# jialeli1/From-Voxel-to-Point

Hardware: AMD Instinct MI355X
Metric: point clouds/sec fwd+bwd (FV2P, KITTI shape) at 1/2/4/8 MI355X (higher is better)
Workload: dtype f32

## Files before the change

### from-voxel-to-point_amd/csrc_torch/fv2p_torch.cpp

```cpp
#include <torch/extension.h>
#include <c10/hip/HIPStream.h>
#include <c10/hip/HIPGuard.h>
#include <c10/hip/HIPCachingAllocator.h>
#include <c10/core/DeviceGuard.h>
#include <hip/hip_runtime_api.h>

#include <atomic>
#include <cstdlib>

#include <map>
#include <tuple>
#include <vector>
#include <mutex>
#include <string>

#include "../../include/fv2p_ops.h"

namespace {

using torch::autograd::AutogradContext;
using torch::autograd::variable_list;

void* cur_stream(const at::Tensor& t) { return static_cast<void*>(c10::hip::getCurrentHIPStream(t.device().index()).stream()); }

// ... 443 lines not shown
    }
    ctx->save_for_backward({x, mean, invstd, weight.has_value() ? *weight : at::Tensor(), bias.has_value() ? *bias : at::Tensor()});
    ctx->saved_data["relu"] = relu;
    ctx->saved_data["batch_stats"] = batch_stats;
    return y;
  }

  static variable_list backward(AutogradContext* ctx, variable_list grads) {
    const auto saved = ctx->get_saved_variables();
    const at::Tensor &x = saved[0], &mean = saved[1], &invstd = saved[2], &weight = saved[3], &bias = saved[4];
    const at::Tensor dz = grads[0].contiguous();
    const int64_t n = x.size(0), c = x.size(1), hw = x.size(2) * x.size(3);
    c10::DeviceGuard guard(x.device());
    void* stream = cur_stream(x);
    at::Tensor dx = at::empty_like(x);
    at::Tensor dpar = at::empty({2, c}, x.options());
    at::Tensor ws = workspace(fv2p_batchnorm2d_ws_bytes(n, static_cast<int>(c), hw), x, stream);
    check(fv2p_batchnorm2d_backward(x.data_ptr<float>(), dz.data_ptr<float>(), n, static_cast<int>(c), hw, mean.data_ptr<float>(), invstd.data_ptr<float>(),
                                    weight.defined() ? weight.data_ptr<float>() : nullptr, bias.defined() ? bias.data_ptr<float>() : nullptr,
                                    ctx->saved_data["relu"].toBool() ? 1 : 0, ctx->saved_data["batch_stats"].toBool() ? 1 : 0, dx.data_ptr<float>(),
                                    dpar[0].data_ptr<float>(), dpar[1].data_ptr<float>(), ws.data_ptr(), static_cast<size_t>(ws.numel()), stream),
          "fv2p_batchnorm2d_backward");
    return {dx, weight.defined() ? dpar[0] : at::Tensor(), bias.defined() ? dpar[1] : at::Tensor(), at::Tensor(), at::Tensor(), at::Tensor(),
            at::Tensor(), at::Tensor(), at::Tensor(), at::Tensor()};
  }
};

at::Tensor batch_norm2d_relu(const at::Tensor& x, const c10::optional<at::Tensor>& weight, const c10::optional<at::Tensor>& bias,
                             const c10::optional<at::Tensor>& running_mean, const c10::optional<at::Tensor>& running_var,
                             const c10::optional<at::Tensor>& num_batches_tracked, bool training, double momentum, double eps, bool relu) {
  return BnRelu2dFn::apply(x, weight, bias, running_mean, running_var, num_batches_tracked, training, momentum, eps, relu);
}

at::Tensor sparse_conv_bn_relu(const at::Tensor& features, const at::Tensor& weight, const at::Tensor& tab_f, int64_t flip_f, const at::Tensor& tab_b,
                               int64_t flip_b, int64_t n_out, int64_t centre, const c10::optional<at::Tensor>& pairs,
                               const c10::optional<at::Tensor>& pair_num, int64_t side_src, const c10::optional<at::Tensor>& conv_bias,
                               const c10::optional<at::Tensor>& bn_weight, const c10::optional<at::Tensor>& bn_bias,
                               const c10::optional<at::Tensor>& running_mean, const c10::optional<at::Tensor>& running_var,
                               const c10::optional<at::Tensor>& num_batches_tracked, bool training, double momentum, double eps, bool relu,
                               const c10::optional<at::Tensor>& perm_b) {
  if (n_out < 2 && training) return at::Tensor();
  const bool has_bias = conv_bias.has_value() && conv_bias->defined();
  const bool batch_stats = training || !(running_mean.has_value() && running_mean->defined());
  const int64_t cout = weight.size(-1);
  if (fuse_bn_stats() && batch_stats && !has_bias && cout <= 1024 && features.is_cuda()) {
    c10::DeviceGuard guard(features.device());
    StatRing& ring = stat_ring(features, cur_stream(features));
    const int cur = ring.cur, other = 1 - cur;
    at::Tensor y = SparseConvFn::apply(features, weight, tab_f, flip_f, tab_b, flip_b, n_out, centre, pairs, pair_num, side_src,
                                       c10::optional<at::Tensor>(ring.buf[cur]), perm_b);
    ring.dirty[cur] = static_cast<int64_t>(fv2p_sparse_conv_stat_slots()) * 2 * cout;
    at::Tensor out = BnReluFn::apply(y, bn_weight, bn_bias, running_mean, running_var, num_batches_tracked, training, momentum, eps, relu,
                                     c10::optional<at::Tensor>(ring.buf[cur]), c10::optional<at::Tensor>(ring.buf[other]), ring.dirty[other]);
    ring.dirty[other] = 0;
    ring.cur = other;
    return out;
  }
  at::Tensor y = SparseConvFn::apply(features, weight, tab_f, flip_f, tab_b, flip_b, n_out, centre, pairs, pair_num, side_src, c10::optional<at::Tensor>(),
                                     perm_b);
  if (has_bias) y = y + *conv_bias;
  return BnReluFn::apply(y, bn_weight, bn_bias, running_mean, running_var, num_batches_tracked, training, momentum, eps, relu,
                         c10::optional<at::Tensor>(), c10::optional<at::Tensor>(), 0);
}


struct FinState {
// ... 494 lines not shown
  m.def("abi_version", []() { return fv2p_abi_version(); });
  m.def("set_bn_epilogue", &set_bn_epilogue, "BatchNorm sums from the conv epilogues (default) or from BatchNorm's own reduce pass");
  m.def("gate_weights", &gate_weights, "aliases of the conv weights whose gradients are joined from the side stream at the end of backward");
  m.def("sparse_conv", &sparse_conv, "fused sparse convolution with autograd (tables from a Rulebook)");
  m.def("batch_norm_relu", &batch_norm_relu, "BatchNorm1d (+ReLU) on [N, C] with autograd");
  m.def("batch_norm2d_relu", &batch_norm2d_relu, "BatchNorm2d (+ReLU) on a contiguous [N, C, H, W] map with autograd");
  m.def("voxelize_batch_mean", &voxelize_batch_mean, py::arg("clouds"), py::arg("voxel_size"), py::arg("range_lo"), py::arg("grid"),
        py::arg("max_points"), py::arg("max_voxels"), py::arg("cloud_streams") = true, py::call_guard<py::gil_scoped_release>(),
        "voxelise a batch of clouds + MeanVFE + collate, without the GIL");
  m.def("build_rulebook_chain", &build_rulebook_chain, py::call_guard<py::gil_scoped_release>(),
        "build a chain of rulebooks (and pair lists) from root coordinates, without the GIL");
  m.def("conv_fin", &conv_fin, "sparse conv with its BatchNorm statistics finalised by the launch (and optionally the source rows' BatchNorm + ReLU on the gather) -> [y, saved]");
  m.def("bn_apply", &bn_apply, "relu?((x - mean) * invstd * gamma + beta [+ residual]) with finalised statistics, one launch");
  m.def("prenorm_supported", &prenorm_supported, "the conv kernel of this shape can normalise its source rows on the gather");
  m.def("set_bn_fold", &set_bn_fold, "round-6 arrangement of conv / BatchNorm / residual blocks on (default) or off (the round-5 one)");
  m.def("bn_fold", &bn_fold);
  m.def("set_deterministic", &set_deterministic, "deterministic mode: no float-atomic conv-epilogue statistics (BatchNorm's own fixed-order reduce)");
  m.def("deterministic", &deterministic);
  m.def("set_bn_one", &set_bn_one, "BatchNorm passes without conv-epilogue sums as one launch each (default) or as reduce + apply");
  m.def("bn_one", &bn_one);
  m.def("set_bn_wide", &set_bn_wide, "large BatchNorm passes with the wide reduce finalised by its own launch (default) or the <= 64-workgroup reduce + folding apply");
  m.def("bn_wide", &bn_wide);
  m.def("record_entry_points", [](bool on) {
    std::lock_guard<std::mutex> lock(g_record_mu);
    g_entries.clear();
    g_record.store(on);
  }, "log the name of every library entry point the binding calls (tests), and clear the log");
  m.def("entry_points", []() {
    std::lock_guard<std::mutex> lock(g_record_mu);
    std::vector<std::string> out;
    out.swap(g_entries);
    return out;
  }, "the entry points called since the last collection");
  m.def("sparse_conv_bn_relu", &sparse_conv_bn_relu, "sparse conv -> BatchNorm1d (-> ReLU) with autograd, one call per backbone block");
}
```

### from-voxel-to-point_amd/fv2p_harness/fv2p_model.py

```python
import math
import os
from functools import partial

import numpy as np
import torch
import torch.nn as nn
import torch.nn.functional as F

from pcdet.ops.iou3d_nms import iou3d_nms_cuda, iou3d_nms_utils
from pcdet.ops.pointnet2.pointnet2_batch import pointnet2_modules as pn2_batch_modules
from pcdet.ops.pointnet2.pointnet2_batch import fused as pn2_fused
from pcdet.ops.pointnet2.pointnet2_batch import pointnet2_utils as pn2_batch
from pcdet.ops.pointnet2.pointnet2_stack import pointnet2_utils as pn2_stack
from pcdet.ops.roiaware_pool3d import roiaware_pool3d_utils
from pcdet.ops.roipoint_pool3d import roipoint_pool3d_utils
from pcdet.models.backbones_3d.pfe import bev_grid_pooling
from pcdet.ops.spconv import norm as _norm

import fv2p_native as _nat

from .backbone import VoxelResBackBone8x, bn_act

TWO_PI = 2.0 * math.pi


class FV2PConfig:
    point_cloud_range = (0.0, -40.0, -3.0, 70.4, 40.0, 1.0)
    voxel_size = (0.05, 0.05, 0.1)
    grid_size = (1408, 1600, 40)
    max_points_per_voxel, max_voxels = 5, 16000
    num_point_features = 4
    bev_layers, bev_strides, bev_filters = (5, 5), (1, 2), (128, 256)
    bev_up_strides, bev_up_filters = (1, 2), (256, 256)
    anchor_rotations = (0.0, 1.57)
    anchor_classes = (((3.9, 1.6, 1.56), -1.78, 0.6, 0.45), ((0.8, 0.6, 1.73), -0.6, 0.5, 0.35), ((1.76, 0.6, 1.73), -0.6, 0.5, 0.35))
    dir_offset, dir_limit_offset, num_dir_bins = 0.78539, 0.0, 2
    rpn_w = dict(cls=1.0, loc=2.0, dir=0.2)
    num_keypoints = 16384
    decode_levels = (("x_conv4", 8, 128, 256), ("x_conv3", 4, 64, 192), ("x_conv2", 2, 32, 160), ("x_conv1", 1, 16, 128))
    init_source, init_stride, init_channels = "x_conv4", 8, 128
    decoder_out = 128
    point_cls_fc, gt_extra_width, point_cls_weight = (64, 64), (0.2, 0.2, 0.2), 4.0
    nms_pre, nms_post, nms_thresh = 9000, 512, 0.8
    roi_per_image, fg_ratio = 128, 0.5
# ... 437 lines not shown

    def __init__(self, cfg, cin):
        super().__init__()
        self.cfg = cfg
        self.cls_layers = mlp1d(cin, cfg.point_cls_fc, out=1)

    @torch.no_grad()
    def assign(self, key, gt):
        boxes = gt[..., :7].contiguous()
        ext = boxes.clone()
        ext[..., 3:6] += dconst(boxes, tuple(float(v) for v in self.cfg.gt_extra_width), boxes.dtype)
        ext = torch.where((boxes[..., 3:6].abs().sum(-1, keepdim=True) > 0), ext, boxes)
        inside = roiaware_pool3d_utils.points_in_boxes_gpu(key, boxes) >= 0
        near = roiaware_pool3d_utils.points_in_boxes_gpu(key, ext) >= 0
        labels = inside.long()
        labels.masked_fill_(inside ^ near, -1)
        return labels.view(-1)

    def forward(self, key, feats, gt):
        logits = run_rows(self.cls_layers, feats)
        labels = self.assign(key, gt)
        pos = labels > 0
        w = ((labels == 0) | pos).float() / pos.sum().float().clamp_min(1.0)
        loss = sigmoid_focal(logits, pos.float().unsqueeze(-1), w).sum() * self.cfg.point_cls_weight
        return loss, torch.sigmoid(logits).max(dim=-1).values


def rows_linear(x, weight, bias=None):
    w = weight.reshape(weight.shape[0], -1).t().unsqueeze(0).expand(x.shape[0], -1, -1)
    y = torch.bmm(x, w)
    return y if bias is None else y + bias


def sa_msg_grid(sa, xyz, features, centres, rows=None):
    outs = []
    xyz_t = xyz.transpose(1, 2)
    ctr_t = centres.transpose(1, 2)
    for grouper, mlp in zip(sa.groupers, sa.mlps):
        layers = list(mlp)
        w1 = layers[0].weight[:, :, 0, 0]
        idx = pn2_batch.ball_query(grouper.radius, grouper.nsample, xyz, centres)
        tail = layers[1:]
        fusable = (len(tail) == 3 and isinstance(tail[0], nn.ReLU) and isinstance(tail[1], nn.Conv2d) and isinstance(tail[2], nn.ReLU)
                   and tail[1].bias is None and tail[1].weight.shape[:2] == (w1.shape[0], w1.shape[0]) and xyz.is_cuda)
        if fusable:
            if rows is None:
                rows = features.transpose(1, 2).contiguous()
            per_point = rows_linear(rows, w1[:, 3:]) + rows_linear(xyz, w1[:, :3])
            per_centre = rows_linear(centres, w1[:, :3])
            if pn2_fused.supported(per_point, idx):
                outs.append(pn2_fused.sa_grid_max(per_point, per_centre, idx, tail[1].weight[:, :, 0, 0]).transpose(1, 2))
                continue
        if features is None:
            features = rows.transpose(1, 2).contiguous()
        per_point = (torch.matmul(w1[:, 3:], features) + torch.matmul(w1[:, :3], xyz_t)).contiguous()
        per_centre = torch.matmul(w1[:, :3], ctr_t)
        h = pn2_batch.grouping_operation(per_point, idx) - per_centre.unsqueeze(-1)
        for layer in tail:
            h = layer(h)
        outs.append(h.amax(dim=-1))
    return torch.cat(outs, dim=1)


class IoUGuidedRoIHead(nn.Module):

    def __init__(self, cfg):
        super().__init__()
        self.cfg = cfg
        self.bev_grid_pool_layer = bev_grid_pooling.BEVGridPooling(
            type("Cfg", (), dict(IN_CHANNELS=cfg.bev_pool_in, OUT_CHANNELS=cfg.bev_pool_out))(), cfg.point_cloud_range, cfg.voxel_size)
        self.roipoint_pool3d_layer = roipoint_pool3d_utils.RoIPointPool3d(cfg.num_sampled_points, list(cfg.pool_extra_width))
        chans = [5] + list(cfg.xyz_up)
        up = []
        for a, c in zip(chans[:-1], chans[1:]):
            up += [nn.Conv2d(a, c, 1), nn.ReLU()]
        self.xyz_up_layer = nn.Sequential(*up)
        c_out = cfg.xyz_up[-1]
        self.merge_down_layer = nn.Sequential(nn.Conv2d(2 * c_out, c_out, 1), nn.ReLU())
        self.SA_modules = nn.ModuleList([pn2_batch_modules.PointnetSAModuleMSG(
            npoint=cfg.grid_size_roi ** 3, radii=list(cfg.sa_radii), nsamples=list(cfg.sa_nsamples),
            mlps=[[c_out] + list(m) for m in cfg.sa_mlps], use_xyz=True, bn=False)])
        sa_out = sum(m[-1] for m in cfg.sa_mlps)
        g3 = cfg.grid_size_roi ** 3
        layers, pre = [], g3 * (sa_out + cfg.bev_pool_out)
        for k, f in enumerate(cfg.interact_filters):
            layers += [nn.Conv1d(pre, f, 1, bias=False), nn.BatchNorm1d(f), nn.ReLU()]
            if k != len(cfg.interact_filters) - 1 and cfg.dp_ratio > 0:
                layers.append(nn.Dropout(cfg.dp_ratio))
# ... 144 lines not shown

    def prepare(self, bev, prop_scores, prop_boxes, gt, uniforms):
        b = bev.shape[0]
        rois, _ = self.proposals(prop_scores, prop_boxes)
        s_rois, s_gt, s_iou = self.sample_targets(rois, gt, uniforms)
        gt_ct = self.canonical_targets(s_rois, s_gt)
        return dict(rois=rois, s_rois=s_rois, s_gt=s_gt, s_iou=s_iou, gt_ct=gt_ct, **self.roi_streams(bev, s_rois))

    def roi_streams(self, bev, s_rois, bev_stride=8):
        b = bev.shape[0]
        world, local = self.grid_points(s_rois)
        batch_dict = {"batch_size": b, "spatial_features_before_head": bev, "spatial_features_stride": bev_stride}
        g = self.cfg.grid_size_roi
        if KERNEL_GLUE and world.shape[1] == g ** 3:
            column = world.view(world.shape[0], g * g, g, 3)[:, :, 0]
            g_bev = self.bev_grid_pool_layer(batch_dict, column.reshape(b, -1, 3))
            g_bev = g_bev.view(world.shape[0], g * g, 1, -1).expand(-1, -1, g, -1).reshape(world.shape[0], g ** 3, -1)
        else:
            g_bev = self.bev_grid_pool_layer(batch_dict, world.view(b, -1, 3)).view(world.shape[0], world.shape[1], -1)
        g_bev = g_bev.permute(0, 2, 1).contiguous()
        t = dconst(s_rois, _CORNER_SIGNS, s_rois.dtype) / 2
        corners = s_rois.reshape(-1, 7)[:, None, 3:6] * t[None]
        cge = self.cge_inter(self.cge_up(corners.transpose(1, 2).unsqueeze(3).contiguous()).squeeze(-1))
        return dict(local=local, g_bev=g_bev, cge=cge)

    def finish(self, key, feats, scores, prep):
        rois = prep["s_rois"]
        cls, reg = self.predict(key, feats, scores, rois, prep)
        loss = self.losses(rois, prep["s_gt"], prep["gt_ct"], prep["s_iou"], cls, reg[:, 1:], reg[:, :1])
        return loss, {"rois": prep["rois"], "sampled_rois": rois, "roi_iou": prep["s_iou"]}

    def predict(self, key, feats, scores, rois, prep):
        pooled = self.pool_points(key, feats, scores, rois)
        h = pooled[..., 0:5]
        for layer in self.xyz_up_layer:
            h = rows_linear(h, layer.weight, layer.bias) if isinstance(layer, nn.Conv2d) else layer(h)
        h = torch.cat((h, pooled[..., 5:]), dim=2)
        for layer in self.merge_down_layer:
            h = rows_linear(h, layer.weight, layer.bias) if isinstance(layer, nn.Conv2d) else layer(h)
        g_pt = sa_msg_grid(self.SA_modules[0], pooled[..., 0:3].contiguous(), None, prep["local"].contiguous(), rows=h)
        grid = torch.cat((g_pt, prep["g_bev"]), dim=1)
        pc = self.grid_interact_fc_layer(grid.view(grid.shape[0], -1, 1))
        shared = self.feature_fusion(torch.cat((pc, prep["cge"]), dim=1))
        cls = self.cls_layers(shared).squeeze(-1)
        reg = self.reg_layers(shared).squeeze(-1)
        return cls, reg

    @staticmethod
    def reg_losses(rois, gt_src, gt_ct, fg, reg):
        n_fg = fg.sum().clamp_min(1.0)
        r7 = rois.reshape(-1, 7)
        anchor = torch.cat((torch.zeros_like(r7[:, :3]), r7[:, 3:6], torch.zeros_like(r7[:, 6:7])), dim=1)
        target = residual_encode(gt_ct.reshape(-1, gt_ct.shape[-1])[:, :7], anchor)
        loss_reg = (smooth_l1(reg - target, 1.0 / 9.0) * fg[:, None]).sum() / n_fg
        local = residual_decode(reg, anchor)
        world = rotate_z(local.unsqueeze(1), r7[:, 6]).squeeze(1)
        world = torch.cat((world[:, :3] + r7[:, :3], world[:, 3:6], world[:, 6:7] + r7[:, 6:7]), dim=1)
        g = gt_src.reshape(-1, gt_src.shape[-1])[:, :7]
        loss_corner = (corner_loss_lidar(world, g) * fg).sum() / n_fg
        return loss_reg, loss_corner

    def losses(self, rois, gt_src, gt_ct, iou, cls, reg, iou_pred):
        cfg = self.cfg
        iou = iou.view(-1)
        soft = ((iou - cfg.cls_bg) / (cfg.cls_fg - cfg.cls_bg)).clamp(0, 1)
        soft = torch.where(iou > cfg.cls_fg, torch.ones_like(soft), torch.where(iou < cfg.cls_bg, torch.zeros_like(soft), soft))
        loss_cls = F.binary_cross_entropy(torch.sigmoid(cls.view(-1)), soft, reduction="none").mean()
        fg = (iou > cfg.reg_fg).float()
        loss_reg, loss_corner = self.reg_losses(rois, gt_src, gt_ct, fg, reg)
        lab = (iou - 0.5) * 2
        valid = (lab >= (cfg.reg_fg - 0.5) * 2).float()
        loss_iou = (F.smooth_l1_loss(iou_pred.view(-1), lab, reduction="none") * valid).sum() / valid.sum().clamp_min(1.0)
        return loss_cls + loss_reg + loss_corner + loss_iou
# ... 95 lines not shown
```

### include/fv2p_ops.h

```cpp
#ifndef FV2P_OPS_H_
#define FV2P_OPS_H_

#include <stddef.h>
#include <stdint.h>

#ifdef __cplusplus
extern "C" {
#endif

#define FV2P_ABI_VERSION 1

#define FV2P_EINVAL      (-1)
#define FV2P_EWORKSPACE  (-2)
#define FV2P_EHIP        (-3)
#define FV2P_ELIMIT      (-4)

typedef void* fv2p_stream_t;

const char* fv2p_last_error(void);
int fv2p_abi_version(void);

size_t fv2p_scan_ws_bytes(int64_t n);
int fv2p_exclusive_scan_i32(const int* in, int* out, int64_t n, int* total, void* ws, size_t ws_bytes,
                            fv2p_stream_t stream);
// ... 267 lines not shown
                                   void* ws, size_t ws_bytes, fv2p_stream_t stream);
size_t fv2p_group_points_stack_grad_ws_bytes(int m, int c, int nsample);
int fv2p_group_points_stack_grad_gather(int b, int m, int c, int n, int nsample, const float* grad_out, const int* idx,
                                        const int* idx_batch_cnt, const int* features_batch_cnt, float* grad_features, void* ws,
                                        size_t ws_bytes, fv2p_stream_t stream);
size_t fv2p_three_interpolate_batch_grad_ws_bytes(int b, int c, int n, int m);
int fv2p_three_interpolate_batch_grad_gather(int b, int c, int n, int m, const float* grad_out, const int* idx, const float* weight,
                                             float* grad_points, void* ws, size_t ws_bytes, fv2p_stream_t stream);

int fv2p_group_points_stack_h(int b, int m, int c, int n, int nsample, const void* features, const int* features_batch_cnt,
                              const int* idx, const int* idx_batch_cnt, void* out, int dtype, fv2p_stream_t stream);
size_t fv2p_group_points_stack_grad_h_ws_bytes(int m, int c, int nsample);
int fv2p_group_points_stack_grad_h(int b, int m, int c, int n, int nsample, const void* grad_out, const int* idx,
                                   const int* idx_batch_cnt, const int* features_batch_cnt, void* grad_features, int dtype,
                                   void* ws, size_t ws_bytes, fv2p_stream_t stream);
int fv2p_three_interpolate_stack_h(int n, int c, int m, const void* features, const int* idx, const float* weight, void* out,
                                   int dtype, fv2p_stream_t stream);
size_t fv2p_three_interpolate_stack_grad_h_ws_bytes(int n, int c, int m);
int fv2p_three_interpolate_stack_grad_h(int n, int c, int m, const void* grad_out, const int* idx, const float* weight,
                                        void* grad_features, int dtype, void* ws, size_t ws_bytes, fv2p_stream_t stream);

int fv2p_sa_grid_supported(int n, int m, int s, int c);
int fv2p_sa_grid_fwd(const float* per_point, const float* per_centre, const int* idx, const float* w2, int rois, int n, int m,
                     int s, int c, float* out, unsigned char* arg, fv2p_stream_t stream);
size_t fv2p_sa_grid_bwd_ws_bytes(int rois);
int fv2p_sa_grid_bwd(const float* per_point, const float* per_centre, const int* idx, const float* w2, const unsigned char* arg,
                     const float* grad_out, int rois, int n, int m, int s, int c, float* grad_point, float* grad_centre,
                     float* grad_w2, void* ws, size_t ws_bytes, fv2p_stream_t stream);
size_t fv2p_sa_grid_bwd_gather_ws_bytes(int rois, int m, int s);
int fv2p_sa_grid_bwd_gather(const float* per_point, const float* per_centre, const int* idx, const float* w2, const unsigned char* arg,
                            const float* grad_out, int rois, int n, int m, int s, int c, float* grad_point, float* grad_centre,
                            float* grad_w2, void* ws, size_t ws_bytes, fv2p_stream_t stream);

int fv2p_dcn_forward(const float* x_nhwc, const float* wt_oc, const float* bias, const float* offset,
                     const float* mask, int batch, int height, int width, int c_in, int c_out, int h_out,
                     int w_out, int kh, int kw, int sh, int sw, int ph, int pw, int dh, int dw,
                     int deformable_group, float* y_nhwc, fv2p_stream_t stream);
int fv2p_dcn_set_forward_order(int order);
int fv2p_dcn_set_colg_cap(int64_t bytes);
size_t fv2p_dcn_backward_ws_bytes(int batch, int height, int width, int h_out, int w_out, int c_in, int c_out, int kh,
                                  int kw, int deformable_group);
int fv2p_dcn_backward(const float* x_nhwc, const float* wt, const float* offset, const float* mask,
                      const float* dy_nhwc, int batch, int height, int width, int c_in, int c_out, int h_out,
                      int w_out, int kh, int kw, int sh, int sw, int ph, int pw, int dh, int dw,
                      int deformable_group, float* dx_nhwc, float* doffset, float* dmask, float* dwt, void* ws,
                      size_t ws_bytes, fv2p_stream_t stream);
int fv2p_dcn_forward_grouped(const float* x_nhwc, const float* wt_oc, const float* bias, const float* offset,
                             const float* mask, int batch, int height, int width, int c_in, int c_out, int h_out,
                             int w_out, int kh, int kw, int sh, int sw, int ph, int pw, int dh, int dw,
                             int deformable_group, int group, float* y_nhwc, fv2p_stream_t stream);
size_t fv2p_dcn_backward_grouped_ws_bytes(int batch, int height, int width, int h_out, int w_out, int c_in, int c_out, int kh,
                                          int kw, int deformable_group, int group);
int fv2p_dcn_backward_grouped(const float* x_nhwc, const float* wt, const float* offset, const float* mask,
                              const float* dy_nhwc, int batch, int height, int width, int c_in, int c_out, int h_out,
                              int w_out, int kh, int kw, int sh, int sw, int ph, int pw, int dh, int dw,
                              int deformable_group, int group, float* dx_nhwc, float* doffset, float* dmask, float* dwt,
                              void* ws, size_t ws_bytes, fv2p_stream_t stream);

int fv2p_transpose_batched(const float* in, int batch, int64_t rows, int64_t cols, float* out, fv2p_stream_t stream);

int fv2p_deform_psroi_pool_forward(const float* data, const float* rois, const float* trans, int batch, int channels,
                                   int height, int width, int num_rois, int no_trans, float spatial_scale,
                                   int output_dim, int group_size, int pooled_size, int part_size,
                                   int sample_per_part, float trans_std, int num_classes, float* out,
                                   float* top_count, fv2p_stream_t stream);
int fv2p_deform_psroi_pool_backward(const float* grad_out, const float* data, const float* rois, const float* trans,
// ... 90 lines not shown
```

Measured before the change: 105.1.

## Fuse RoI point MLP stack and SA first layers into one MFMA kernel

Adds a HIP kernel pair that runs the RoI-head point MLP chain (xyz_up two layers, merge_down, and both SA-branch first 1x1 convs) per 64-row tile in LDS using fp32 MFMA, with a fused backward that computes all weight and bias gradients via per-block partials and a reduction kernel. The model's predict path uses it when the layer shapes match and feeds the per-point outputs straight into the SA grid op. This removes several bmm launches and the intermediate activation tensors' round trips to memory. In exchange it adds weight-fragment packing per call, a fixed-shape specialization, and a change in gradient summation order.

```diff
diff --git a/from-voxel-to-point_amd/csrc/roi_mlp.hip b/from-voxel-to-point_amd/csrc/roi_mlp.hip
--- /dev/null
+++ b/from-voxel-to-point_amd/csrc/roi_mlp.hip
@@ -0,0 +1,476 @@
+#include "common.hpp"
+
+namespace fv2p {
+namespace {
+
+typedef float f32x4 __attribute__((ext_vector_type(4)));
+
+constexpr int kRmC = 128;
+constexpr int kRmIn = 5 + kRmC;
+constexpr int kRmS = 64;
+constexpr int kRmSLd = 3 + kRmC;
+constexpr int kRmT = 64;
+constexpr int kRmThreads = 512;
+constexpr int kRmParts = 240;
+constexpr int kRmLdF = 132;
+constexpr int kRmLdB = 144;
+
+constexpr int kFragW2 = 0;
+constexpr int kFragW3a = 16384;
+constexpr int kFragW3b = 32768;
+constexpr int kFragS0 = 49152;
+constexpr int kFragS1 = 57344;
+constexpr int kFragFwd = 65536;
+constexpr int kFragS0T = 65536;
+constexpr int kFragS1T = 73728;
+constexpr int kFragW3aT = 81920;
+constexpr int kFragW2T = 98304;
+constexpr int kFragBwd = 114688;
+
+constexpr int kGradW1 = 0;
+constexpr int kGradB1 = 640;
+constexpr int kGradW2 = 768;
+constexpr int kGradB2 = 17152;
+constexpr int kGradW3 = 17280;
+constexpr int kGradB3 = 50048;
+constexpr int kGradS0 = 50176;
+constexpr int kGradS1 = 58560;
+constexpr int kGradFloats = 66944;
+
+struct PackJob {
+  const float* src;
+  int ld, col0, transpose, nb, nj, dst;
+};
+struct PackJobs {
+  PackJob job[9];
+};
+
+__global__ __launch_bounds__(256) void roi_mlp_pack_k(PackJobs jobs, float* __restrict__ image) {
+  const PackJob d = jobs.job[blockIdx.y];
+  const int e = blockIdx.x * 256 + threadIdx.x;
+  if (e >= d.nb * d.nj * 64) return;
+  const int lane = e & 63, bj = e >> 6, b = bj / d.nj, j = bj - b * d.nj;
+  const int i = 16 * b + (lane & 15), k = 16 * j + 4 * (lane >> 4);
+  float v[4];
+#pragma unroll
+  for (int c = 0; c < 4; ++c) v[c] = d.transpose ? d.src[(k + c) * d.ld + d.col0 + i] : d.src[i * d.ld + d.col0 + k + c];
+  *reinterpret_cast<float4*>(image + d.dst + static_cast<size_t>(e) * 4) = make_float4(v[0], v[1], v[2], v[3]);
+}
+
+template <int NBW, int NJ, int UJ, typename X>
+__device__ __forceinline__ void mma_rows(const float* __restrict__ frag, int b0, int lane, X x, f32x4 (&acc)[NBW]) {
+#pragma unroll UJ
+  for (int j = 0; j < NJ; ++j) {
+    const float4 xv = x(j);
+    float4 a[NBW];
+#pragma unroll
+    for (int i = 0; i < NBW; ++i)
+      a[i] = *reinterpret_cast<const float4*>(frag + ((b0 + i) * NJ + j) * 256 + static_cast<unsigned>(lane * 4));
+#pragma unroll
+    for (int i = 0; i < NBW; ++i) acc[i] = __builtin_amdgcn_mfma_f32_16x16x4f32(a[i].x, xv.x, acc[i], 0, 0, 0);
+#pragma unroll
+    for (int i = 0; i < NBW; ++i) acc[i] = __builtin_amdgcn_mfma_f32_16x16x4f32(a[i].y, xv.y, acc[i], 0, 0, 0);
+#pragma unroll
+    for (int i = 0; i < NBW; ++i) acc[i] = __builtin_amdgcn_mfma_f32_16x16x4f32(a[i].z, xv.z, acc[i], 0, 0, 0);
+#pragma unroll
+    for (int i = 0; i < NBW; ++i) acc[i] = __builtin_amdgcn_mfma_f32_16x16x4f32(a[i].w, xv.w, acc[i], 0, 0, 0);
+  }
+}
+
+template <int N>
+__device__ __forceinline__ void zero_acc(f32x4 (&acc)[N]) {
+#pragma unroll
+  for (int i = 0; i < N; ++i) acc[i] = f32x4{0.f, 0.f, 0.f, 0.f};
+}
+
+template <int NBW>
+__device__ __forceinline__ void layer1_row(const float (&x)[5], const float* __restrict__ w1, const float* __restrict__ b1, int b0, int g,
+                                           float* __restrict__ dst) {
+#pragma unroll
+  for (int i = 0; i < NBW; ++i) {
+    const int c0 = 16 * (b0 + i) + 4 * g;
+    float v[4];
+#pragma unroll
+    for (int e = 0; e < 4; ++e) {
+      const float* w = w1 + static_cast<unsigned>((c0 + e) * 5);
+      float z = x[0] * w[0];
+      z = fmaf(x[1], w[1], z);
+      z = fmaf(x[2], w[2], z);
+      z = fmaf(x[3], w[3], z);
+      z = fmaf(x[4], w[4], z);
+      v[e] = fmaxf(z + b1[static_cast<unsigned>(c0 + e)], 0.f);
+    }
+    *reinterpret_cast<float4*>(dst + c0) = make_float4(v[0], v[1], v[2], v[3]);
+  }
+}
+
+template <int NBW>
+__device__ __forceinline__ void store_relu(const f32x4 (&acc)[NBW], const float* __restrict__ bias, int b0, int g, float* __restrict__ dst) {
+#pragma unroll
+  for (int i = 0; i < NBW; ++i) {
+    const int c0 = 16 * (b0 + i) + 4 * g;
+    const float4 b = *reinterpret_cast<const float4*>(bias + static_cast<unsigned>(c0));
+    *reinterpret_cast<float4*>(dst + c0) =
+        make_float4(fmaxf(acc[i][0] + b.x, 0.f), fmaxf(acc[i][1] + b.y, 0.f), fmaxf(acc[i][2] + b.z, 0.f), fmaxf(acc[i][3] + b.w, 0.f));
+  }
+}
+
+__global__ __launch_bounds__(kRmThreads, 4) void roi_point_mlp_fwd_k(long long rows, const float* __restrict__ pooled,
+                                                                      const float* __restrict__ w1, const float* __restrict__ b1,
+                                                                      const float* __restrict__ b2, const float* __restrict__ b3,
+                                                                      const float* __restrict__ s0, const float* __restrict__ s1,
+                                                                      const float* __restrict__ frag, float* __restrict__ out0,
+                                                                      float* __restrict__ out1) {
+  __shared__ __attribute__((aligned(16))) float bufa[kRmT * kRmLdF];
+  __shared__ __attribute__((aligned(16))) float bufb[kRmT * kRmLdF];
+  const int lane = threadIdx.x & 63, wave = threadIdx.x >> 6, row = lane & 15, g = lane >> 4;
+  const int rt = wave & 3, hb = wave >> 2, lr = 16 * rt + row;
+  const long long r0 = static_cast<long long>(blockIdx.x) * kRmT;
+  const bool valid = r0 + lr < rows;
+  const float* prow = pooled + (valid ? r0 + lr : rows - 1) * kRmIn;
+  float x[5];
+#pragma unroll
+  for (int d = 0; d < 5; ++d) x[d] = prow[d];
+  float* la = bufa + lr * kRmLdF;
+  float* lb = bufb + lr * kRmLdF;
+  layer1_row<4>(x, w1, b1, 4 * hb, g, la);
+  __syncthreads();
+  f32x4 acc[4];
+  zero_acc(acc);
+  mma_rows<4, 8, 8>(frag + kFragW2, 4 * hb, lane, [&](int j) { return *reinterpret_cast<const float4*>(la + 16 * j + 4 * g); }, acc);
+  store_relu(acc, b2, 4 * hb, g, lb);
+  __syncthreads();
+  zero_acc(acc);
+  mma_rows<4, 8, 8>(frag + kFragW3a, 4 * hb, lane, [&](int j) { return *reinterpret_cast<const float4*>(lb + 16 * j + 4 * g); }, acc);
+  mma_rows<4, 8, 8>(frag + kFragW3b, 4 * hb, lane, [&](int j) {
+    const float* p = prow + 5 + 16 * j + 4 * g;
+    return make_float4(p[0], p[1], p[2], p[3]);
+  }, acc);
+  store_relu(acc, b3, 4 * hb, g, la);
+  __syncthreads();
+  zero_acc(acc);
+  mma_rows<4, 8, 8>(frag + (hb ? kFragS1 : kFragS0), 0, lane, [&](int j) { return *reinterpret_cast<const float4*>(la + 16 * j + 4 * g); }, acc);
+  if (valid) {
+    const float* sk = hb ? s1 : s0;
+    float* o = (hb ? out1 : out0) + (r0 + lr) * kRmS;
+#pragma unroll
+    for (int i = 0; i < 4; ++i) {
+      const int c0 = 16 * i + 4 * g;
+      float v[4];
+#pragma unroll
+      for (int e = 0; e < 4; ++e) {
+        const float* w = sk + (c0 + e) * kRmSLd;
+        float t = x[0] * w[0];
+        t = fmaf(x[1], w[1], t);
+        t = fmaf(x[2], w[2], t);
+        v[e] = acc[i][e] + t;
+      }
+      *reinterpret_cast<float4*>(o + c0) = make_float4(v[0], v[1], v[2], v[3]);
+    }
+  }
+}
+
+template <int NT, int UT, int NA, typename GV, typename AV>
+__device__ __forceinline__ void wgrad_rows(GV gv, AV av, f32x4 (&acc)[NA]) {
+  static_assert(NT <= NA, "more column blocks than accumulators");
+#pragma unroll UT
+  for (int t = 0; t < kRmT / 4; ++t) {
+    const float gval = gv(t);
+#pragma unroll
+    for (int n = 0; n < NT; ++n) acc[n] = __builtin_amdgcn_mfma_f32_16x16x4f32(gval, av(t, n), acc[n], 0, 0, 0);
+  }
+}
+
+constexpr int kRmBwdThreads = 1024;
+__global__ __launch_bounds__(kRmBwdThreads) void roi_point_mlp_bwd_k(long long rows, int tiles, const float* __restrict__ pooled,
+                                                                      const float* __restrict__ dp0, const float* __restrict__ dp1,
+                                                                      const float* __restrict__ w1, const float* __restrict__ b1,
+                                                                      const float* __restrict__ b2, const float* __restrict__ b3,
+                                                                      const float* __restrict__ frag, float* __restrict__ partial) {
+  __shared__ __attribute__((aligned(16))) float buf1[kRmT * kRmLdB];
+  __shared__ __attribute__((aligned(16))) float buf2[kRmT * kRmLdB];
+  __shared__ __attribute__((aligned(16))) float buf3[kRmT * kRmLdB];
+  __shared__ __attribute__((aligned(16))) float buff[kRmT * kRmLdB];
+  __shared__ __attribute__((aligned(16))) float bufx[kRmT * 16];
+  __shared__ __attribute__((aligned(16))) float wsm[5 * kRmC + 3 * kRmC];
+  __shared__ float dbs[3 * kRmC];
+  const int tid = threadIdx.x;
+  if (tid < 5 * kRmC) wsm[tid] = w1[tid];
+  if (tid < kRmC) {
+    wsm[5 * kRmC + tid] = b1[tid];
+    wsm[6 * kRmC + tid] = b2[tid];
+    wsm[7 * kRmC + tid] = b3[tid];
+  }
+  f32x4 aw3[8], aw2[4], as[5], aw1[1];
+  zero_acc(aw3);
+  zero_acc(aw2);
+  zero_acc(as);
+  zero_acc(aw1);
+  if (tid < 3 * kRmC) dbs[tid] = 0.f;
+
+  for (int tile = blockIdx.x; tile < tiles; tile += gridDim.x) {
+    int tv = tid;
+    asm volatile("" : "+v"(tv));
+    const int lane = tv & 63, row = lane & 15, g = lane >> 4;
+    const int wave = __builtin_amdgcn_readfirstlane(tv >> 6);
+    const int rt = wave & 3, b0 = 2 * (wave >> 2), lr = 16 * rt + row;
+    const int bi = wave & 7, half = wave >> 3;
+    const float* dpk = (bi >> 2) ? dp1 : dp0;
+    float* l1 = buf1 + lr * kRmLdB;
+    float* l2 = buf2 + lr * kRmLdB;
+    float* l3 = buf3 + lr * kRmLdB;
+    const float* lf = buff + lr * kRmLdB;
+    const int go = g * kRmLdB + row;
+    const long long r0 = static_cast<long long>(tile) * kRmT;
+    const bool valid = r0 + lr < rows;
+    const long long last = rows - 1;
+    const float* prow = pooled + (valid ? r0 + lr : last) * kRmIn;
+    for (int e = tv; e < kRmT * kRmC; e += kRmBwdThreads) {
+      const int rr = e >> 7, c = e & 127;
+      const long long gr = r0 + rr < rows ? r0 + rr : last;
+      buff[rr * kRmLdB + c] = pooled[gr * kRmIn + 5 + c];
+    }
+    {
+      const int rr = tv >> 4, c = tv & 15;
+      const long long gr = r0 + rr < rows ? r0 + rr : last;
+      bufx[tv] = c < 5 ? pooled[gr * kRmIn + c] : 0.f;
+    }
+    float x[5];
+#pragma unroll
+    for (int d = 0; d < 5; ++d) x[d] = prow[d];
+    int wo = 0;
+    asm volatile("" : "+v"(wo));
+    const float* fr = frag;
+    asm volatile("" : "+s"(fr));
+    const float *w1t = wsm + wo, *b1t = w1t + 5 * kRmC, *b2t = w1t + 6 * kRmC, *b3t = w1t + 7 * kRmC;
+    __syncthreads();
+    layer1_row<2>(x, w1t, b1t, b0, g, l1);
+    __syncthreads();
+    f32x4 acc[2];
+    zero_acc(acc);
+    mma_rows<2, 8, 2>(fr + kFragW2, b0, lane, [&](int j) { return *reinterpret_cast<const float4*>(l1 + 16 * j + 4 * g); }, acc);
+    store_relu(acc, b2t, b0, g, l2);
+    __syncthreads();
+    zero_acc(acc);
+    mma_rows<2, 8, 2>(fr + kFragW3a, b0, lane, [&](int j) { return *reinterpret_cast<const float4*>(l2 + 16 * j + 4 * g); }, acc);
+    mma_rows<2, 8, 2>(fr + kFragW3b, b0, lane, [&](int j) { return *reinterpret_cast<const float4*>(lf + 16 * j + 4 * g); }, acc);
+    store_relu(acc, b3t, b0, g, l3);
+    __syncthreads();
+    {
+      auto gv = [&](int t) {
+        const long long gr = r0 + 4 * t + g;
+        return gr < rows ? dpk[gr * kRmS + 16 * (bi & 3) + row] : 0.f;
+      };
+      wgrad_rows<5, 2>(gv, [&](int t, int n) { return n < 4 ? buf3[(4 * t) * kRmLdB + go + 16 * (4 * half + n)] : bufx[(4 * t + g) * 16 + row]; }, as);
+    }
+    zero_acc(acc);
+    {
+      const float* d0 = dp0 + (r0 + lr) * kRmS + 4 * g;
+      const float* d1 = dp1 + (r0 + lr) * kRmS + 4 * g;
+      const float4 zero = make_float4(0.f, 0.f, 0.f, 0.f);
+      mma_rows<2, 4, 2>(fr + kFragS0T, b0, lane, [&](int j) { return valid ? *reinterpret_cast<const float4*>(d0 + 16 * j) : zero; }, acc);
+      mma_rows<2, 4, 2>(fr + kFragS1T, b0, lane, [&](int j) { return valid ? *reinterpret_cast<const float4*>(d1 + 16 * j) : zero; }, acc);
+    }
+    float4 dz[2];
+#pragma unroll
+    for (int i = 0; i < 2; ++i) {
+      const float4 a = *reinterpret_cast<const float4*>(l3 + 16 * (b0 + i) + 4 * g);
+      dz[i] = make_float4(a.x > 0.f ? acc[i][0] : 0.f, a.y > 0.f ? acc[i][1] : 0.f, a.z > 0.f ? acc[i][2] : 0.f, a.w > 0.f ? acc[i][3] : 0.f);
+    }
+    __syncthreads();
+#pragma unroll
+    for (int i = 0; i < 2; ++i) *reinterpret_cast<float4*>(l3 + 16 * (b0 + i) + 4 * g) = dz[i];
+    __syncthreads();
+    if (tv < kRmC) {
+      float s = 0.f;
+#pragma unroll 8
+      for (int rr = 0; rr < kRmT; ++rr) s += buf3[rr * kRmLdB + tv];
+      dbs[2 * kRmC + tv] += s;
+    }
+    {
+      const float* a2f = half ? buff : buf2;
+      wgrad_rows<8, 2>([&](int t) { return buf3[(4 * t) * kRmLdB + go + 16 * bi]; }, [&](int t, int n) { return a2f[(4 * t) * kRmLdB + go + 16 * n]; }, aw3);
+    }
+    zero_acc(acc);
+    mma_rows<2, 8, 2>(fr + kFragW3aT, b0, lane, [&](int j) { return *reinterpret_cast<const float4*>(l3 + 16 * j + 4 * g); }, acc);
+#pragma unroll
+    for (int i = 0; i < 2; ++i) {
+      const float4 a = *reinterpret_cast<const float4*>(l2 + 16 * (b0 + i) + 4 * g);
+      dz[i] = make_float4(a.x > 0.f ? acc[i][0] : 0.f, a.y > 0.f ? acc[i][1] : 0.f, a.z > 0.f ? acc[i][2] : 0.f, a.w > 0.f ? acc[i][3] : 0.f);
+    }
+    __syncthreads();
+#pragma unroll
+    for (int i = 0; i < 2; ++i) *reinterpret_cast<float4*>(l2 + 16 * (b0 + i) + 4 * g) = dz[i];
+    __syncthreads();
+    if (tv < kRmC) {
+      float s = 0.f;
+#pragma unroll 8
+      for (int rr = 0; rr < kRmT; ++rr) s += buf2[rr * kRmLdB + tv];
+      dbs[kRmC + tv] += s;
+    }
+    wgrad_rows<4, 2>([&](int t) { return buf2[(4 * t) * kRmLdB + go + 16 * bi]; },
+                     [&](int t, int n) { return buf1[(4 * t) * kRmLdB + go + 16 * (4 * half + n)]; }, aw2);
+    zero_acc(acc);
+    mma_rows<2, 8, 2>(fr + kFragW2T, b0, lane, [&](int j) { return *reinterpret_cast<const float4*>(l2 + 16 * j + 4 * g); }, acc);
+#pragma unroll
+    for (int i = 0; i < 2; ++i) {
+      const float4 a = *reinterpret_cast<const float4*>(l1 + 16 * (b0 + i) + 4 * g);
+      dz[i] = make_float4(a.x > 0.f ? acc[i][0] : 0.f, a.y > 0.f ? acc[i][1] : 0.f, a.z > 0.f ? acc[i][2] : 0.f, a.w > 0.f ? acc[i][3] : 0.f);
+    }
+    __syncthreads();
+#pragma unroll
+    for (int i = 0; i < 2; ++i) *reinterpret_cast<float4*>(l1 + 16 * (b0 + i) + 4 * g) = dz[i];
+    __syncthreads();
+    if (tv < kRmC) {
+      float s = 0.f;
+#pragma unroll 8
+      for (int rr = 0; rr < kRmT; ++rr) s += buf1[rr * kRmLdB + tv];
+      dbs[tv] += s;
+    }
+    if (half == 0)
+      wgrad_rows<1, 4>([&](int t) { return buf1[(4 * t) * kRmLdB + go + 16 * bi]; }, [&](int t, int) { return bufx[(4 * t + g) * 16 + row]; }, aw1);
+    __syncthreads();
+  }
+
+  const int lane = tid & 63, row = lane & 15, g = lane >> 4, wave = tid >> 6, bi = wave & 7, half = wave >> 3;
+  float* out = partial + static_cast<size_t>(blockIdx.x) * kGradFloats;
+#pragma unroll
+  for (int n = 0; n < 8; ++n)
+#pragma unroll
+    for (int e = 0; e < 4; ++e) out[kGradW3 + (16 * bi + 4 * g + e) * (2 * kRmC) + 16 * (8 * half + n) + row] = aw3[n][e];
+#pragma unroll
+  for (int n = 0; n < 4; ++n)
+#pragma unroll
+    for (int e = 0; e < 4; ++e) out[kGradW2 + (16 * bi + 4 * g + e) * kRmC + 16 * (4 * half + n) + row] = aw2[n][e];
+  float* os = out + ((bi >> 2) ? kGradS1 : kGradS0);
+#pragma unroll
+  for (int n = 0; n < 4; ++n)
+#pragma unroll
+    for (int e = 0; e < 4; ++e) os[(16 * (bi & 3) + 4 * g + e) * kRmSLd + 3 + 16 * (4 * half + n) + row] = as[n][e];
+  if (half == 0 && row < 3) {
+#pragma unroll
+    for (int e = 0; e < 4; ++e) os[(16 * (bi & 3) + 4 * g + e) * kRmSLd + row] = as[4][e];
+  }
+  if (half == 0 && row < 5) {
+#pragma unroll
+    for (int e = 0; e < 4; ++e) out[kGradW1 + (16 * bi + 4 * g + e) * 5 + row] = aw1[0][e];
+  }
+  if (tid < kRmC) {
+    out[kGradB1 + tid] = dbs[tid];
+    out[kGradB2 + tid] = dbs[kRmC + tid];
+    out[kGradB3 + tid] = dbs[2 * kRmC + tid];
+  }
+}
+
+struct GradOuts {
+  float* p[8];
+};
+
+__global__ __launch_bounds__(256) void roi_mlp_grad_reduce_k(int parts, const float* __restrict__ partial, GradOuts outs) {
+  __shared__ float group[4][64];
+  const int el = threadIdx.x & 63, q = threadIdx.x >> 6;
+  const int e = blockIdx.x * 64 + el;
+  const int per = (parts + 3) / 4;
+  const int p1 = (q + 1) * per < parts ? (q + 1) * per : parts;
+  float s = 0.f;
+  if (e < kGradFloats)
+    for (int p = q * per; p < p1; ++p) s += partial[static_cast<size_t>(p) * kGradFloats + e];
+  group[q][el] = s;
+  __syncthreads();
+  if (q != 0 || e >= kGradFloats) return;
+  s = ((group[0][el] + group[1][el]) + group[2][el]) + group[3][el];
+  constexpr int off[9] = {kGradW1, kGradB1, kGradW2, kGradB2, kGradW3, kGradB3, kGradS0, kGradS1, kGradFloats};
+  int seg = 0;
+#pragma unroll
+  for (int k = 1; k < 8; ++k) seg += e >= off[k] ? 1 : 0;
+  int base = 0;
+#pragma unroll
+  for (int k = 1; k < 8; ++k) base = e >= off[k] ? off[k] : base;
+  outs.p[seg][e - base] = s;
+}
+
+int pack_images(const float* w2, const float* w3, const float* s0, const float* s1, bool backward, float* image, hipStream_t stream) {
+  PackJobs jobs;
+  jobs.job[0] = {w2, kRmC, 0, 0, 8, 8, kFragW2};
+  jobs.job[1] = {w3, 2 * kRmC, 0, 0, 8, 8, kFragW3a};
+  jobs.job[2] = {w3, 2 * kRmC, kRmC, 0, 8, 8, kFragW3b};
+  jobs.job[3] = {s0, kRmSLd, 3, 0, 4, 8, kFragS0};
+  jobs.job[4] = {s1, kRmSLd, 3, 0, 4, 8, kFragS1};
+  jobs.job[5] = {s0, kRmSLd, 3, 1, 8, 4, kFragS0T};
+  jobs.job[6] = {s1, kRmSLd, 3, 1, 8, 4, kFragS1T};
+  jobs.job[7] = {w3, 2 * kRmC, 0, 1, 8, 8, kFragW3aT};
+  jobs.job[8] = {w2, kRmC, 0, 1, 8, 8, kFragW2T};
+  hipLaunchKernelGGL(roi_mlp_pack_k, dim3(8 * 8 * 64 / 256, backward ? 9 : 5), dim3(256), 0, stream, jobs, image);
+  FV2P_LAUNCH_CHECK();
+  return 0;
+}
+
+bool rows_ok(int64_t rows) { return rows >= 1 && rows <= (1ll << 30); }
+int bwd_parts(int64_t rows) { return static_cast<int>(ceil_div(rows, kRmT) < kRmParts ? ceil_div(rows, kRmT) : kRmParts); }
+
+}
+}
+
+using namespace fv2p;
+
+extern "C" int fv2p_roi_point_mlp_supported(int c, int up0, int up1, int merge, int sa0, int sa1) {
+  return c == kRmC && up0 == kRmC && up1 == kRmC && merge == kRmC && sa0 == kRmS && sa1 == kRmS;
+}
+
+extern "C" size_t fv2p_roi_point_mlp_fwd_ws_bytes(int64_t rows) {
+  (void)rows;
+  Sizer sz;
+  sz.take<float>(kFragFwd);
+  return sz.bytes();
+}
+
+extern "C" int fv2p_roi_point_mlp_fwd(const float* pooled, int64_t rows, const float* w_up0, const float* b_up0, const float* w_up1,
+                                      const float* b_up1, const float* w_merge, const float* b_merge, const float* w_sa0,
+                                      const float* w_sa1, float* per_point0, float* per_point1, void* ws, size_t ws_bytes,
+                                      fv2p_stream_t stream_) {
+  FV2P_REQUIRE(rows_ok(rows), FV2P_EINVAL, "roi_point_mlp_fwd: needs 1 .. 2^30 rows");
+  FV2P_REQUIRE(pooled && w_up0 && b_up0 && w_up1 && b_up1 && w_merge && b_merge && w_sa0 && w_sa1 && per_point0 && per_point1, FV2P_EINVAL,
+               "roi_point_mlp_fwd: null pointer");
+  FV2P_REQUIRE(ws && ws_bytes >= fv2p_roi_point_mlp_fwd_ws_bytes(rows), FV2P_EWORKSPACE, "roi_point_mlp_fwd: workspace too small");
+  hipStream_t stream = static_cast<hipStream_t>(stream_);
+  Carver cv(ws, ws_bytes);
+  float* image = cv.take<float>(kFragFwd);
+  if (int rc = pack_images(w_up1, w_merge, w_sa0, w_sa1, false, image, stream)) return rc;
+  hipLaunchKernelGGL(roi_point_mlp_fwd_k, dim3(static_cast<unsigned>(ceil_div(rows, kRmT))), dim3(kRmThreads), 0, stream,
+                     static_cast<long long>(rows), pooled, w_up0, b_up0, b_up1, b_merge, w_sa0, w_sa1, image, per_point0, per_point1);
+  FV2P_LAUNCH_CHECK();
+  return 0;
+}
+
+extern "C" size_t fv2p_roi_point_mlp_bwd_ws_bytes(int64_t rows) {
+  Sizer sz;
+  sz.take<float>(kFragBwd);
+  sz.take<float>(static_cast<size_t>(rows_ok(rows) ? bwd_parts(rows) : 1) * kGradFloats);
+  return sz.bytes();
+}
+
+extern "C" int fv2p_roi_point_mlp_bwd(const float* pooled, int64_t rows, const float* grad0, const float* grad1, const float* w_up0,
+                                      const float* b_up0, const float* w_up1, const float* b_up1, const float* w_merge,
+                                      const float* b_merge, const float* w_sa0, const float* w_sa1, float* g_w_up0, float* g_b_up0,
+                                      float* g_w_up1, float* g_b_up1, float* g_w_merge, float* g_b_merge, float* g_w_sa0, float* g_w_sa1,
+                                      void* ws, size_t ws_bytes, fv2p_stream_t stream_) {
+  FV2P_REQUIRE(rows_ok(rows), FV2P_EINVAL, "roi_point_mlp_bwd: needs 1 .. 2^30 rows");
+  FV2P_REQUIRE(pooled && grad0 && grad1 && w_up0 && b_up0 && w_up1 && b_up1 && w_merge && b_merge && w_sa0 && w_sa1, FV2P_EINVAL,
+               "roi_point_mlp_bwd: null pointer");
+  FV2P_REQUIRE(g_w_up0 && g_b_up0 && g_w_up1 && g_b_up1 && g_w_merge && g_b_merge && g_w_sa0 && g_w_sa1, FV2P_EINVAL,
+               "roi_point_mlp_bwd: null gradient pointer");
+  FV2P_REQUIRE(ws && ws_bytes >= fv2p_roi_point_mlp_bwd_ws_bytes(rows), FV2P_EWORKSPACE, "roi_point_mlp_bwd: workspace too small");
+  hipStream_t stream = static_cast<hipStream_t>(stream_);
+  const int parts = bwd_parts(rows);
+  Carver cv(ws, ws_bytes);
+  float* image = cv.take<float>(kFragBwd);
+  float* partial = cv.take<float>(static_cast<size_t>(parts) * kGradFloats);
+  if (int rc = pack_images(w_up1, w_merge, w_sa0, w_sa1, true, image, stream)) return rc;
+  hipLaunchKernelGGL(roi_point_mlp_bwd_k, dim3(parts), dim3(kRmBwdThreads), 0, stream, static_cast<long long>(rows),
+                     static_cast<int>(ceil_div(rows, kRmT)), pooled, grad0, grad1, w_up0, b_up0, b_up1, b_merge, image, partial);
+  FV2P_LAUNCH_CHECK();
+  GradOuts outs{{g_w_up0, g_b_up0, g_w_up1, g_b_up1, g_w_merge, g_b_merge, g_w_sa0, g_w_sa1}};
+  hipLaunchKernelGGL(roi_mlp_grad_reduce_k, dim3(ceil_div(kGradFloats, 64)), dim3(256), 0, stream, parts, partial, outs);
+  FV2P_LAUNCH_CHECK();
+  return 0;
+}
diff --git a/from-voxel-to-point_amd/csrc_torch/fv2p_torch.cpp b/from-voxel-to-point_amd/csrc_torch/fv2p_torch.cpp
--- a/from-voxel-to-point_amd/csrc_torch/fv2p_torch.cpp
+++ b/from-voxel-to-point_amd/csrc_torch/fv2p_torch.cpp
@@ -499,6 +499,65 @@
   return BnRelu2dFn::apply(x, weight, bias, running_mean, running_var, num_batches_tracked, training, momentum, eps, relu);
 }
 
+struct RoiPointMlpFn : public torch::autograd::Function<RoiPointMlpFn> {
+  static variable_list forward(AutogradContext* ctx, const at::Tensor& pooled_, at::TensorList params_) {
+    TORCH_CHECK(params_.size() == 8, "roi_point_mlp: eight parameters expected");
+    require_f32_cuda(pooled_, "roi_point_mlp pooled");
+    TORCH_CHECK(pooled_.dim() == 3 && pooled_.numel() > 0, "roi_point_mlp: pooled must be (R, N, 5 + C)");
+    c10::DeviceGuard guard(pooled_.device());
+    at::Tensor pooled = pooled_.contiguous();
+    variable_list params;
+    for (const auto& p : params_) {
+      require_f32_cuda(p, "roi_point_mlp parameter");
+      params.push_back(p.contiguous());
+    }
+    const int64_t rows = pooled.size(0) * pooled.size(1);
+    at::Tensor out0 = at::empty({pooled.size(0), pooled.size(1), 64}, pooled.options());
+    at::Tensor out1 = at::empty_like(out0);
+    void* stream = cur_stream(pooled);
+    const size_t need = fv2p_roi_point_mlp_fwd_ws_bytes(rows);
+    at::Tensor ws = workspace(need, pooled, stream);
+    const float* w[8];
+    for (int i = 0; i < 8; ++i) w[i] = params[i].data_ptr<float>();
+    check(fv2p_roi_point_mlp_fwd(pooled.data_ptr<float>(), rows, w[0], w[1], w[2], w[3], w[4], w[5], w[6], w[7], out0.data_ptr<float>(),
+                                 out1.data_ptr<float>(), ws.data_ptr(), static_cast<size_t>(ws.numel()), stream),
+          "fv2p_roi_point_mlp_fwd");
+    variable_list keep{pooled};
+    keep.insert(keep.end(), params.begin(), params.end());
+    ctx->save_for_backward(keep);
+    return {out0, out1};
+  }
+  static variable_list backward(AutogradContext* ctx, variable_list grads) {
+    auto saved = ctx->get_saved_variables();
+    const at::Tensor& pooled = saved[0];
+    c10::DeviceGuard guard(pooled.device());
+    const int64_t rows = pooled.size(0) * pooled.size(1);
+    at::Tensor g[2];
+    for (int k = 0; k < 2; ++k)
+      g[k] = grads[k].defined() ? grads[k].contiguous() : at::zeros({pooled.size(0), pooled.size(1), 64}, pooled.options());
+    variable_list out{at::Tensor()};
+    const float* w[8];
+    float* d[8];
+    for (int i = 0; i < 8; ++i) {
+      out.push_back(at::empty_like(saved[1 + i]));
+      w[i] = saved[1 + i].data_ptr<float>();
+      d[i] = out.back().data_ptr<float>();
+    }
+    void* stream = cur_stream(pooled);
+    const size_t need = fv2p_roi_point_mlp_bwd_ws_bytes(rows);
+    at::Tensor ws = workspace(need, pooled, stream);
+    check(fv2p_roi_point_mlp_bwd(pooled.data_ptr<float>(), rows, g[0].data_ptr<float>(), g[1].data_ptr<float>(), w[0], w[1], w[2], w[3], w[4],
+                                 w[5], w[6], w[7], d[0], d[1], d[2], d[3], d[4], d[5], d[6], d[7], ws.data_ptr(),
+                                 static_cast<size_t>(ws.numel()), stream),
+          "fv2p_roi_point_mlp_bwd");
+    return out;
+  }
+};
+
+std::vector<at::Tensor> roi_point_mlp(const at::Tensor& pooled, const std::vector<at::Tensor>& params) {
+  return RoiPointMlpFn::apply(pooled, at::TensorList(params));
+}
+
 at::Tensor sparse_conv_bn_relu(const at::Tensor& features, const at::Tensor& weight, const at::Tensor& tab_f, int64_t flip_f, const at::Tensor& tab_b,
                                int64_t flip_b, int64_t n_out, int64_t centre, const c10::optional<at::Tensor>& pairs,
                                const c10::optional<at::Tensor>& pair_num, int64_t side_src, const c10::optional<at::Tensor>& conv_bias,
@@ -1059,5 +1118,6 @@
     out.swap(g_entries);
     return out;
   }, "the entry points called since the last collection");
+  m.def("roi_point_mlp", &roi_point_mlp, "pooled-point MLP chain of the RoI head with autograd: (pooled, [8 parameters]) -> [per_point_0, per_point_1]");
   m.def("sparse_conv_bn_relu", &sparse_conv_bn_relu, "sparse conv -> BatchNorm1d (-> ReLU) with autograd, one call per backbone block");
 }
diff --git a/from-voxel-to-point_amd/fv2p_harness/fv2p_model.py b/from-voxel-to-point_amd/fv2p_harness/fv2p_model.py
--- a/from-voxel-to-point_amd/fv2p_harness/fv2p_model.py
+++ b/from-voxel-to-point_amd/fv2p_harness/fv2p_model.py
@@ -10,6 +10,7 @@
 from pcdet.ops.iou3d_nms import iou3d_nms_cuda, iou3d_nms_utils
 from pcdet.ops.pointnet2.pointnet2_batch import pointnet2_modules as pn2_batch_modules
 from pcdet.ops.pointnet2.pointnet2_batch import fused as pn2_fused
+from pcdet.ops.pointnet2.pointnet2_batch import roi_mlp as pn2_roi_mlp
 from pcdet.ops.pointnet2.pointnet2_batch import pointnet2_utils as pn2_batch
 from pcdet.ops.pointnet2.pointnet2_stack import pointnet2_utils as pn2_stack
 from pcdet.ops.roiaware_pool3d import roiaware_pool3d_utils
@@ -513,11 +514,11 @@
     return y if bias is None else y + bias
 
 
-def sa_msg_grid(sa, xyz, features, centres, rows=None):
+def sa_msg_grid(sa, xyz, features, centres, rows=None, per_points=None):
     outs = []
     xyz_t = xyz.transpose(1, 2)
     ctr_t = centres.transpose(1, 2)
-    for grouper, mlp in zip(sa.groupers, sa.mlps):
+    for k, (grouper, mlp) in enumerate(zip(sa.groupers, sa.mlps)):
         layers = list(mlp)
         w1 = layers[0].weight[:, :, 0, 0]
         idx = pn2_batch.ball_query(grouper.radius, grouper.nsample, xyz, centres)
@@ -525,16 +526,22 @@
         fusable = (len(tail) == 3 and isinstance(tail[0], nn.ReLU) and isinstance(tail[1], nn.Conv2d) and isinstance(tail[2], nn.ReLU)
                    and tail[1].bias is None and tail[1].weight.shape[:2] == (w1.shape[0], w1.shape[0]) and xyz.is_cuda)
         if fusable:
-            if rows is None:
-                rows = features.transpose(1, 2).contiguous()
-            per_point = rows_linear(rows, w1[:, 3:]) + rows_linear(xyz, w1[:, :3])
+            if per_points is not None:
+                per_point = per_points[k]
+            else:
+                if rows is None:
+                    rows = features.transpose(1, 2).contiguous()
+                per_point = rows_linear(rows, w1[:, 3:]) + rows_linear(xyz, w1[:, :3])
             per_centre = rows_linear(centres, w1[:, :3])
             if pn2_fused.supported(per_point, idx):
                 outs.append(pn2_fused.sa_grid_max(per_point, per_centre, idx, tail[1].weight[:, :, 0, 0]).transpose(1, 2))
                 continue
-        if features is None:
-            features = rows.transpose(1, 2).contiguous()
-        per_point = (torch.matmul(w1[:, 3:], features) + torch.matmul(w1[:, :3], xyz_t)).contiguous()
+        if per_points is not None:
+            per_point = per_points[k].transpose(1, 2).contiguous()
+        else:
+            if features is None:
+                features = rows.transpose(1, 2).contiguous()
+            per_point = (torch.matmul(w1[:, 3:], features) + torch.matmul(w1[:, :3], xyz_t)).contiguous()
         per_centre = torch.matmul(w1[:, :3], ctr_t)
         h = pn2_batch.grouping_operation(per_point, idx) - per_centre.unsqueeze(-1)
         for layer in tail:
@@ -745,6 +752,13 @@
 
     def predict(self, key, feats, scores, rois, prep):
         pooled = self.pool_points(key, feats, scores, rois)
+        sa = self.SA_modules[0]
+        if KERNEL_GLUE and pn2_roi_mlp.enabled() and pn2_roi_mlp.supported(pooled, self.xyz_up_layer, self.merge_down_layer, [m[0] for m in sa.mlps]):
+            up, md = self.xyz_up_layer, self.merge_down_layer
+            per_points = pn2_roi_mlp.roi_point_mlp(pooled, up[0].weight, up[0].bias, up[2].weight, up[2].bias, md[0].weight, md[0].bias,
+                                                   sa.mlps[0][0].weight, sa.mlps[1][0].weight)
+            g_pt = sa_msg_grid(sa, pooled[..., 0:3].contiguous(), None, prep["local"].contiguous(), per_points=per_points)
+            return self.heads(g_pt, prep)
         h = pooled[..., 0:5]
         for layer in self.xyz_up_layer:
             h = rows_linear(h, layer.weight, layer.bias) if isinstance(layer, nn.Conv2d) else layer(h)
@@ -752,6 +766,9 @@
         for layer in self.merge_down_layer:
             h = rows_linear(h, layer.weight, layer.bias) if isinstance(layer, nn.Conv2d) else layer(h)
         g_pt = sa_msg_grid(self.SA_modules[0], pooled[..., 0:3].contiguous(), None, prep["local"].contiguous(), rows=h)
+        return self.heads(g_pt, prep)
+
+    def heads(self, g_pt, prep):
         grid = torch.cat((g_pt, prep["g_bev"]), dim=1)
         pc = self.grid_interact_fc_layer(grid.view(grid.shape[0], -1, 1))
         shared = self.feature_fusion(torch.cat((pc, prep["cge"]), dim=1))
diff --git a/from-voxel-to-point_amd/pcdet/ops/pointnet2/pointnet2_batch/roi_mlp.py b/from-voxel-to-point_amd/pcdet/ops/pointnet2/pointnet2_batch/roi_mlp.py
--- /dev/null
+++ b/from-voxel-to-point_amd/pcdet/ops/pointnet2/pointnet2_batch/roi_mlp.py
@@ -0,0 +1,69 @@
+import torch
+from torch import nn
+
+import fv2p_native as _nat
+
+from ... import _glue as G
+
+_ENABLED = True
+
+
+def set_enabled(on):
+    global _ENABLED
+    _ENABLED = bool(on)
+
+
+def enabled():
+    return _ENABLED
+
+
+def _conv1x1(m, cin, bias):
+    return (type(m) is nn.Conv2d and m.kernel_size == (1, 1) and m.stride == (1, 1) and m.groups == 1 and m.in_channels == cin
+            and (m.bias is not None) == bias and m.weight.dtype == torch.float32 and m.weight.is_cuda)
+
+
+def supported(pooled, xyz_up, merge_down, sa_first):
+    if not (torch.is_tensor(pooled) and pooled.is_cuda and pooled.dtype == torch.float32 and pooled.dim() == 3 and pooled.numel() > 0
+            and not pooled.requires_grad):
+        return False
+    up, md, sa = list(xyz_up), list(merge_down), list(sa_first)
+    c = pooled.shape[2] - 5
+    if not (len(up) == 4 and len(md) == 2 and len(sa) == 2 and isinstance(up[1], nn.ReLU) and isinstance(up[3], nn.ReLU)
+            and isinstance(md[1], nn.ReLU)):
+        return False
+    if not (_conv1x1(up[0], 5, True) and _conv1x1(up[2], up[0].out_channels, True) and _conv1x1(md[0], up[2].out_channels + c, True)
+            and _conv1x1(sa[0], 3 + md[0].out_channels, False) and _conv1x1(sa[1], 3 + md[0].out_channels, False)):
+        return False
+    return bool(_nat.lib().fv2p_roi_point_mlp_supported(c, up[0].out_channels, up[2].out_channels, md[0].out_channels, sa[0].out_channels,
+                                                        sa[1].out_channels))
+
+
+def _fwd(saved, pooled, *params):
+    r, n, _ = pooled.shape
+    rows = r * n
+    pooled = pooled.contiguous()
+    params = tuple(p.contiguous() for p in params)
+    out0, out1 = G.new(pooled, (r, n, 64)), G.new(pooled, (r, n, 64))
+    ws = G.scratch("fv2p_roi_point_mlp_fwd_ws_bytes", pooled.device, rows)
+    G.run("fv2p_roi_point_mlp_fwd", pooled, rows, *params, out0, out1, ws, ws.numel())
+    saved.update(t=(pooled,) + params, rows=rows)
+    return out0, out1
+
+
+def _bwd(saved, grad0, grad1):
+    pooled, *params = saved["t"]
+    rows = saved["rows"]
+    grads = tuple(torch.empty_like(p) for p in params)
+    ws = G.scratch("fv2p_roi_point_mlp_bwd_ws_bytes", pooled.device, rows)
+    G.run("fv2p_roi_point_mlp_bwd", pooled, rows, grad0.contiguous(), grad1.contiguous(), *params, *grads, ws, ws.numel())
+    return (None,) + grads
+
+
+RoiPointMlp = G.autograd_op("RoiPointMlp", _fwd, _bwd)
+
+
+def roi_point_mlp(pooled, w_up0, b_up0, w_up1, b_up1, w_merge, b_merge, w_sa0, w_sa1):
+    ext = _nat.torch_ext()
+    if ext is not None:
+        return tuple(ext.roi_point_mlp(pooled, [w_up0, b_up0, w_up1, b_up1, w_merge, b_merge, w_sa0, w_sa1]))
+    return RoiPointMlp.apply(pooled, w_up0, b_up0, w_up1, b_up1, w_merge, b_merge, w_sa0, w_sa1)
diff --git a/include/fv2p_ops.h b/include/fv2p_ops.h
--- a/include/fv2p_ops.h
+++ b/include/fv2p_ops.h
@@ -323,6 +323,19 @@
                             const float* grad_out, int rois, int n, int m, int s, int c, float* grad_point, float* grad_centre,
                             float* grad_w2, void* ws, size_t ws_bytes, fv2p_stream_t stream);
 
+int fv2p_roi_point_mlp_supported(int c, int up0, int up1, int merge, int sa0, int sa1);
+size_t fv2p_roi_point_mlp_fwd_ws_bytes(int64_t rows);
+int fv2p_roi_point_mlp_fwd(const float* pooled, int64_t rows, const float* w_up0, const float* b_up0, const float* w_up1,
+                           const float* b_up1, const float* w_merge, const float* b_merge, const float* w_sa0,
+                           const float* w_sa1, float* per_point0, float* per_point1, void* ws, size_t ws_bytes,
+                           fv2p_stream_t stream);
+size_t fv2p_roi_point_mlp_bwd_ws_bytes(int64_t rows);
+int fv2p_roi_point_mlp_bwd(const float* pooled, int64_t rows, const float* grad0, const float* grad1, const float* w_up0,
+                           const float* b_up0, const float* w_up1, const float* b_up1, const float* w_merge,
+                           const float* b_merge, const float* w_sa0, const float* w_sa1, float* g_w_up0, float* g_b_up0,
+                           float* g_w_up1, float* g_b_up1, float* g_w_merge, float* g_b_merge, float* g_w_sa0, float* g_w_sa1,
+                           void* ws, size_t ws_bytes, fv2p_stream_t stream);
+
 int fv2p_dcn_forward(const float* x_nhwc, const float* wt_oc, const float* bias, const float* offset,
                      const float* mask, int batch, int height, int width, int c_in, int c_out, int h_out,
                      int w_out, int kh, int kw, int sh, int sw, int ph, int pw, int dh, int dw,
```

Measured after the change: 105.3, median of 3. No clear change (+0.2%).
